# LuChengTHU/dpm-solver

Measured on NVIDIA H100. Metric: solver-update GElem/s, higher is better.
Workload: dtype bf16

## Files before the change

### dpm_solver_b200/_lib.py

```python
from __future__ import annotations

import ctypes as C
import os
from pathlib import Path

_PKG = Path(__file__).resolve().parent
LIB_PATH = _PKG / "lib" / "libdpmsolver_b200.so"

DPM_F32, DPM_BF16, DPM_F16 = 0, 1, 2
FORM_NONE, FORM_LIN1, FORM_LIN2, FORM_LIN3, FORM_DIFF2, FORM_MS3, FORM_SS3T = range(7)
PARAM_NOISE, PARAM_X_START, PARAM_V, PARAM_SCORE = range(4)

PARAM_BY_NAME = {"noise": PARAM_NOISE, "x_start": PARAM_X_START, "v": PARAM_V, "score": PARAM_SCORE}


class StepDesc(C.Structure):
    _fields_ = [
        ("x", C.c_void_p), ("xe", C.c_void_p), ("m0", C.c_void_p), ("m1", C.c_void_p),
        ("m2", C.c_void_p), ("m_out", C.c_void_p), ("out", C.c_void_p), ("out2", C.c_void_p),
        ("e_cond", C.c_void_p), ("e_uncond", C.c_void_p), ("thr", C.c_void_p),
        ("n", C.c_uint64), ("per_sample", C.c_uint64),
        ("state_dtype", C.c_int32), ("model_dtype", C.c_int32), ("form", C.c_int32),
        ("n_model", C.c_int32), ("param", C.c_int32), ("predict_x0", C.c_int32),
        ("c0_on_old", C.c_int32), ("raw_round", C.c_int32),
        ("guidance", C.c_float), ("alpha_e", C.c_float), ("sigma_e", C.c_float),
        ("a", C.c_float), ("c0", C.c_float), ("c1", C.c_float), ("c2", C.c_float),
        ("w0", C.c_float), ("w1", C.c_float), ("w2", C.c_float), ("w3", C.c_float),
        ("w4", C.c_float),
        ("dev_coef", C.c_void_p),
    ]


class AdaptiveCtl(C.Structure):
    _fields_ = [
        ("schedule_kind", C.c_int32), ("table_len", C.c_int32),
        ("t_array", C.c_void_p), ("log_alpha_array", C.c_void_p), ("log_alpha_flipped", C.c_void_p), ("t_flipped", C.c_void_p),
        ("beta_0", C.c_float), ("beta_1_minus_beta_0", C.c_float), ("inv_total_N", C.c_float),
        ("discrete_time_input", C.c_int32), ("order", C.c_int32), ("predict_x0", C.c_int32), ("taylor", C.c_int32),
        ("t_0", C.c_float), ("theta", C.c_float), ("t_err", C.c_float),
        ("state", C.c_void_p), ("coef", C.c_void_p), ("times", C.c_void_p), ("error", C.c_void_p),
    ]


_vp, _f, _u64, _i = C.c_void_p, C.c_float, C.c_uint64, C.c_int

PROTOTYPES = {
    "dpm_version": (C.c_int, []),
    "dpm_last_error": (C.c_char_p, []),
    "dpm_set_tuning": (C.c_int, [_i, _i, _i]),
    "dpm_get_tuning": (C.c_int, [C.POINTER(C.c_int)] * 3),
    "dpm_launch_count": (C.c_uint64, []),
    "dpm_step": (C.c_int, [C.POINTER(StepDesc), _vp]),
    "dpm_lincomb": (C.c_int, [_vp, _vp, _vp, _vp, _vp, _i, _f, _f, _f, _f, _u64, _i, _vp]),
    "dpm_solver_first_update": (C.c_int, [_vp, _vp, _vp, _f, _f, _u64, _i, _vp]),
    "dpm_multistep_second_update": (C.c_int, [_vp, _vp, _vp, _vp, _f, _f, _f, _f, _u64, _i, _vp]),
    "dpm_multistep_third_update": (C.c_int, [_vp] * 5 + [_f] * 8 + [_u64, _i, _vp]),
    "dpm_singlestep_diff_update": (C.c_int, [_vp, _vp, _vp, _vp, _f, _f, _f, _u64, _i, _vp]),
    "dpm_singlestep_third_taylor_update": (C.c_int, [_vp] * 5 + [_f] * 9 + [_u64, _i, _vp]),
    "dpm_cfg_combine": (C.c_int, [_vp, _vp, _vp, _f, _u64, _i, _vp]),
    "dpm_duplicate": (C.c_int, [_vp, _vp, _u64, _i, _vp]),
    "dpm_philox_policy": (C.c_int, [_u64, C.POINTER(C.c_uint32), C.POINTER(C.c_uint64)]),
    "dpm_add_noise_philox": (C.c_int, [_vp, _vp, _u64, _i, C.POINTER(C.c_float), C.POINTER(C.c_float), _u64, _u64, _i, _i, _vp]),
    "dpm_diffedit_corrector": (C.c_int, [_vp, _vp, _vp, _vp, _u64, _u64, _f, _f, _u64, _u64, _i, _vp]),
    "dpm_data_prediction": (C.c_int, [_vp, _vp, _vp, _f, _f, _vp, _u64, _u64, _i, _vp]),
    "dpm_dynamic_threshold_workspace": (C.c_size_t, [_u64, _u64]),
    "dpm_dynamic_threshold": (C.c_int, [_vp, C.POINTER(StepDesc), _f, _f, _vp, C.c_size_t, _vp]),
    "dpm_adaptive_init": (C.c_int, [C.POINTER(AdaptiveCtl), _f, _f, _vp]),
    "dpm_adaptive_plan": (C.c_int, [C.POINTER(AdaptiveCtl), _vp]),
    "dpm_adaptive_decide": (C.c_int, [C.POINTER(AdaptiveCtl), _vp]),
    "dpm_select_copy": (C.c_int, [_vp, _vp, _vp, _u64, _vp]),
    "dpm_adaptive_error_workspace": (C.c_size_t, [_u64, _u64]),
    "dpm_adaptive_error": (C.c_int, [_vp, _vp, _vp, _vp, _f, _f, _u64, _u64, _i, _vp, C.c_size_t, _vp]),
    "dpm_cfg_rescale_workspace": (C.c_size_t, [_u64, _u64]),
    "dpm_cfg_rescale_ratio": (C.c_int, [_vp, _vp, _vp, _f, _u64, _u64, _i, _vp, C.c_size_t, _vp]),
    "dpm_step_rescaled": (C.c_int, [C.POINTER(StepDesc), _vp, _f, _f, _vp]),
}

_lib = None


class DpmLibraryError(RuntimeError):
    pass


def lib() -> C.CDLL:
    global _lib
    if _lib is not None:
        return _lib
    path = Path(os.environ.get("DPM_B200_LIB", LIB_PATH))
    if not path.exists():
        raise DpmLibraryError(
            f"{path} not found. Build it with `python -m dpm_solver_b200.build` "
            "(needs nvcc, sm_90a). dpm_solver_b200 has no CPU or PyTorch fallback.")
    handle = C.CDLL(str(path))
    for name, (res, args) in PROTOTYPES.items():
        try:
            fn = getattr(handle, name)
        except AttributeError as e:
            raise DpmLibraryError(f"{path} does not export {name}") from e
        fn.restype = res
        fn.argtypes = args
    _lib = handle
    return _lib


def check(rc: int) -> None:
    if rc != 0:
        msg = lib().dpm_last_error().decode("utf-8", "replace")
        raise DpmLibraryError(f"libdpmsolver_b200 error {rc}: {msg}")
```

### dpm_solver_b200/csrc/capi.cu

```cuda
#include <atomic>
#include <mutex>
#include <set>
#include <utility>
#include <cstdarg>
#include <cstdio>
#include <cstdlib>
#include <cstring>

#include "launch.cuh"

namespace dpm {

static thread_local char g_err[512] = "";
static std::atomic<uint64_t> g_launches{0};
static std::atomic<int> g_variant{2}, g_threads{0}, g_ctas{0};

void set_error(const char* fmt, ...) {
  va_list ap;
  va_start(ap, fmt);
  vsnprintf(g_err, sizeof(g_err), fmt, ap);
  va_end(ap);
}
void count_launch() { g_launches.fetch_add(1, std::memory_order_relaxed); }
bool pdl_enabled() {
  static const bool on = [] { const char* e = getenv("DPM_PDL"); return !(e && e[0] == '0'); }();
  return on;
}

int launch_error(const char* what, cudaError_t e) {
  set_error("%s: %s", what, cudaGetErrorString(e));
  cudaGetLastError();
  return (int)e;
}

template <cudaDeviceAttr A, int FALLBACK>
static int device_attr() {
  static int cache[64] = {0};
  int dev = 0;
  if (cudaGetDevice(&dev) != cudaSuccess || dev < 0 || dev >= 64) return FALLBACK;
  if (cache[dev] == 0) {
    int v = 0;
    if (cudaDeviceGetAttribute(&v, A, dev) != cudaSuccess || v <= 0) v = FALLBACK;
    cache[dev] = v;
  }
  return cache[dev];
}
int sm_count() { return device_attr<cudaDevAttrMultiProcessorCount, 132>(); }
int max_smem_optin() { return device_attr<cudaDevAttrMaxSharedMemoryPerBlockOptin, 227 * 1024>(); }

int ensure_max_smem(const void* kernel, bool nonportable_cluster) {
  static std::mutex mu;
  static std::set<std::pair<int, const void*>> done;
  int dev = 0;
  cudaGetDevice(&dev);
  std::lock_guard<std::mutex> lock(mu);
  if (done.count({dev, kernel})) return 0;
  cudaFuncAttributes fa;
  cudaError_t e = cudaFuncGetAttributes(&fa, kernel);
  const int room = max_smem_optin() - (e == cudaSuccess ? (int)fa.sharedSizeBytes : 0);
  if (e == cudaSuccess) e = cudaFuncSetAttribute(kernel, cudaFuncAttributeMaxDynamicSharedMemorySize, room);
  if (e == cudaSuccess && nonportable_cluster)
    e = cudaFuncSetAttribute(kernel, cudaFuncAttributeNonPortableClusterSizeAllowed, 1);
  if (e != cudaSuccess) return launch_error("shared-memory opt-in failed", e);
  done.insert({dev, kernel});
  return 0;
}

static inline int esize(int dt) { return dt == DPM_F32 ? 4 : 2; }
static inline bool valid_dtype(int dt) { return dt == DPM_F32 || dt == DPM_BF16 || dt == DPM_F16; }
static inline bool aligned(const void* p, int dt) {
  const uintptr_t a = dt == DPM_F32 ? 32 : 16;
  return (reinterpret_cast<uintptr_t>(p) & (a - 1)) == 0;
}
static inline const void* off(const void* p, int dt, uint64_t elems) {
  return p ? static_cast<const char*>(p) + elems * esize(dt) : nullptr;
}
static inline void* off(void* p, int dt, uint64_t elems) {
  return p ? static_cast<char*>(p) + elems * esize(dt) : nullptr;
}

struct Needs {
  bool x, m0, m1, m2, ec, eu, xe;
};

static int build_params(const dpm_step_desc* d, KParams* kp, Needs* nd, bool for_quantile) {
  if (d == nullptr) { set_error("desc is NULL"); return DPM_ERR_ARG; }
  if (!valid_dtype(d->state_dtype) || !valid_dtype(d->model_dtype)) {
    set_error("bad dtype (state %d, model %d)", d->state_dtype, d->model_dtype);
    return DPM_ERR_ARG;
  }
  const int form = for_quantile ? DPM_FORM_NONE : d->form;
  if (form < DPM_FORM_NONE || form > DPM_FORM_SS3T) { set_error("bad form %d", form); return DPM_ERR_ARG; }
  if (d->n_model < 0 || d->n_model > 2) { set_error("n_model must be 0, 1 or 2"); return DPM_ERR_ARG; }
  if (d->param < DPM_PARAM_NOISE || d->param > DPM_PARAM_SCORE) { set_error("bad param %d", d->param); return DPM_ERR_ARG; }
  if (d->raw_round != 0 && ((d->raw_round & ~7) != 0 || ((d->raw_round & 3) != DPM_BF16 && (d->raw_round & 3) != DPM_F16))) {
    set_error("raw_round must be 0 or (DPM_BF16 | DPM_F16) [+ 4]");
    return DPM_ERR_ARG;
  }
  if (d->raw_round != 0 && (d->state_dtype != DPM_F32 || for_quantile)) {
    set_error("raw_round needs an fp32 state and is not available in dpm_dynamic_threshold");
    return DPM_ERR_ARG;
  }
  if ((d->n >> 3) > 0xffffffffull) { set_error("n too large (max 2^35-1 elements per call)"); return DPM_ERR_ARG; }

  const FormReads reads = form_reads(form);
  nd->x = reads.x;
  nd->m0 = d->n_model == 0;
  nd->m1 = reads.m1;
  nd->m2 = reads.m2;
// ... 57 lines not shown
static bool all_aligned(const KParams& p, const Needs& nd) {
  const int sd = p.state_dtype, md = p.model_dtype;
  bool ok = true;
  if (nd.x) ok &= aligned(p.x, sd);
  if (nd.xe) ok &= aligned(p.xe, sd);
  if (nd.m0) ok &= aligned(p.m0, sd);
  if (nd.m1) ok &= aligned(p.m1, sd);
  if (nd.m2) ok &= aligned(p.m2, sd);
  if (nd.ec) ok &= aligned(p.ec, md);
  if (nd.eu) ok &= aligned(p.eu, md);
  if (p.m_out) ok &= aligned(p.m_out, sd);
  if (p.out) ok &= aligned(p.out, sd);
  if (p.out2) ok &= aligned(p.out2, sd);
  return ok;
}

static KParams shifted(const KParams& p, uint64_t elems) {
  KParams t = p;
  const int sd = p.state_dtype, md = p.model_dtype;
  t.x = off(p.x, sd, elems); t.xe = off(p.xe, sd, elems); t.m0 = off(p.m0, sd, elems);
  t.m1 = off(p.m1, sd, elems); t.m2 = off(p.m2, sd, elems);
  t.ec = off(p.ec, md, elems); t.eu = off(p.eu, md, elems);
  t.m_out = off(p.m_out, sd, elems); t.out = off(p.out, sd, elems); t.out2 = off(p.out2, sd, elems);
  t.n = p.n - elems;
  t.elem_offset = elems;
  return t;
}

static int finish(int rc) {
  if (rc != DPM_OK) return rc;
  cudaError_t e = cudaPeekAtLastError();
  return e != cudaSuccess ? launch_error("CUDA launch failed", e) : DPM_OK;
}

struct Rescale {
  const float* ratio;
  float phi, psi;
};

static int step_impl(const dpm_step_desc* d, cudaStream_t stream, const Rescale* rs = nullptr) {
  KParams p;
  Needs nd;
  if (d != nullptr && d->n == 0) return DPM_OK;
  int rc = build_params(d, &p, &nd, false);
  if (rc != DPM_OK) return rc;
  if (p.n == 0) return DPM_OK;
  if (rs != nullptr) {
    if (rs->ratio == nullptr || d->n_model != 2 || d->raw_round != 0 || d->per_sample == 0 || d->n % d->per_sample) {
      set_error("rescaled step: needs ratio, n_model == 2, raw_round == 0 and per_sample dividing n");
      return DPM_ERR_ARG;
    }
    p.ratio = rs->ratio; p.phi = rs->phi; p.psi = rs->psi;
  }
  Tuning t{g_variant.load(), g_threads.load(), g_ctas.load()};

  bool body_done = false;
  if (p.npk > 0 && all_aligned(p, nd) && p.dev_coef == nullptr) {
    int r = 1;
    const bool tma = p.raw_round == 0 &&
                     p.ratio == nullptr &&
                     t.variant == 1;
    if (tma) r = launch_step_tma(p, t, stream);
    if (r == 1) r = launch_step_direct(p, t, stream);
    if (r < 0 || r > 1) return r;
    body_done = (r == 0);
  }
  if (!body_done) {
    rc = launch_step_scalar(p, stream);
  } else if (p.n % kPacket) {
    rc = launch_step_scalar(shifted(p, (uint64_t)p.npk * kPacket), stream);
  }
  return finish(rc);
}

}

using namespace dpm;

extern "C" {

int dpm_version(void) { return DPM_B200_VERSION; }
const char* dpm_last_error(void) { return g_err; }
uint64_t dpm_launch_count(void) { return g_launches.load(); }

int dpm_set_tuning(int variant, int threads, int ctas_per_sm) {
  if (variant < 0 || variant > 2) { set_error("variant must be 0 (direct), 1 (TMA ring) or 2 (auto)"); return DPM_ERR_ARG; }
  if (threads != 0 && (threads < 32 || threads > 512 || threads % 32)) { set_error("threads must be a multiple of 32 in [32,512]"); return DPM_ERR_ARG; }
  if (ctas_per_sm < 0 || ctas_per_sm > 32) { set_error("ctas_per_sm must be in [0,32]"); return DPM_ERR_ARG; }
  g_variant = variant; g_threads = threads; g_ctas = ctas_per_sm;
  return DPM_OK;
}
int dpm_get_tuning(int* variant, int* threads, int* ctas_per_sm) {
  if (variant) *variant = g_variant.load();
  if (threads) *threads = g_threads.load();
  if (ctas_per_sm) *ctas_per_sm = g_ctas.load();
  return DPM_OK;
}

int dpm_step(const dpm_step_desc* desc, dpm_stream_t stream) {
  return step_impl(desc, static_cast<cudaStream_t>(stream));
}

int dpm_step_rescaled(const dpm_step_desc* desc, const float* ratio, float phi, float one_minus_phi,
                      dpm_stream_t stream) {
  const Rescale rs{ratio, phi, one_minus_phi};
  return step_impl(desc, static_cast<cudaStream_t>(stream), &rs);
}

size_t dpm_cfg_rescale_workspace(uint64_t n_samples, uint64_t per_sample) {
  return cfg_rescale_workspace_bytes(n_samples, per_sample);
}

int dpm_cfg_rescale_ratio(float* ratio_out, const void* e_cond, const void* e_uncond, float guidance,
                          uint64_t per_sample, uint64_t n, int model_dtype, void* workspace, size_t workspace_bytes,
                          dpm_stream_t stream) {
  if (n == 0) return DPM_OK;
  if (!ratio_out || !e_cond || !e_uncond) { set_error("cfg rescale: NULL tensor"); return DPM_ERR_ARG; }
  if (!valid_dtype(model_dtype) || per_sample == 0 || n % per_sample) { set_error("cfg rescale: bad dtype or sizes"); return DPM_ERR_ARG; }
  return finish(launch_cfg_rescale_ratio(ratio_out, e_cond, e_uncond, guidance, per_sample, n, model_dtype, workspace,
                                         workspace_bytes, static_cast<cudaStream_t>(stream)));
}

static dpm_step_desc base_desc(void* out, const void* x, uint64_t n, int dtype, int form) {
  dpm_step_desc d;
  memset(&d, 0, sizeof(d));
  d.out = out; d.x = x; d.n = n; d.state_dtype = dtype; d.model_dtype = dtype; d.form = form;
  return d;
}

int dpm_lincomb(void* out, const void* x, const void* m0, const void* m1, const void* m2, int k,
                float a, float c0, float c1, float c2, uint64_t n, int dtype, dpm_stream_t stream) {
  if (k < 1 || k > 3) { set_error("k must be 1, 2 or 3"); return DPM_ERR_ARG; }
  dpm_step_desc d = base_desc(out, x, n, dtype, k == 1 ? DPM_FORM_LIN1 : k == 2 ? DPM_FORM_LIN2 : DPM_FORM_LIN3);
  d.m0 = m0; d.m1 = m1; d.m2 = m2; d.a = a; d.c0 = c0; d.c1 = c1; d.c2 = c2;
  return dpm_step(&d, stream);
}

int dpm_solver_first_update(void* x_t, const void* x, const void* model_s, float a, float c0,
                            uint64_t n, int dtype, dpm_stream_t stream) {
  dpm_step_desc d = base_desc(x_t, x, n, dtype, DPM_FORM_LIN1);
  d.m0 = model_s; d.a = a; d.c0 = c0;
  return dpm_step(&d, stream);
}

int dpm_multistep_second_update(void* x_t, const void* x, const void* model_prev_0,
                                const void* model_prev_1, float a, float c0, float c1,
                                float inv_r0, uint64_t n, int dtype, dpm_stream_t stream) {
  dpm_step_desc d = base_desc(x_t, x, n, dtype, DPM_FORM_DIFF2);
  d.m0 = model_prev_0; d.m1 = model_prev_1; d.a = a; d.c0 = c0; d.c1 = c1; d.w0 = inv_r0;
  return dpm_step(&d, stream);
}

int dpm_multistep_third_update(void* x_t, const void* x, const void* model_prev_0,
                               const void* model_prev_1, const void* model_prev_2, float a,
                               float c0, float c1, float c2, float inv_r0, float inv_r1, float w,
                               float q, uint64_t n, int dtype, dpm_stream_t stream) {
  dpm_step_desc d = base_desc(x_t, x, n, dtype, DPM_FORM_MS3);
  d.m0 = model_prev_0; d.m1 = model_prev_1; d.m2 = model_prev_2;
  d.a = a; d.c0 = c0; d.c1 = c1; d.c2 = c2; d.w0 = inv_r0; d.w1 = inv_r1; d.w2 = w; d.w3 = q;
  return dpm_step(&d, stream);
}

int dpm_singlestep_diff_update(void* x_t, const void* x, const void* model_s,
                               const void* model_new, float a, float c0, float c1, uint64_t n,
                               int dtype, dpm_stream_t stream) {
  dpm_step_desc d = base_desc(x_t, x, n, dtype, DPM_FORM_DIFF2);
// ... 117 lines not shown
```

### dpm_solver_b200/csrc/common.cuh

```cuda
#pragma once
#include <cuda_bf16.h>
#include <cuda_fp16.h>
#include <cuda_runtime.h>
#include <stdint.h>
#include <string.h>

#include "dpm_solver_b200.h"

namespace dpm {

constexpr int kPacket = 8;

struct KParams {
  const void* x;
  const void* xe;
  const void* m0;
  const void* m1;
  const void* m2;
  const void* ec;
  const void* eu;
  void* m_out;
  void* out;
  void* out2;
  const float* thr;
  uint64_t n;
  uint32_t npk;
  uint32_t pk_per_sample;
  uint64_t per_sample;
  uint64_t elem_offset;
  int32_t param;
  int32_t predict_x0;
  int32_t c0_on_old;
  int32_t use_xe;
  int32_t xe_is_x;
  int32_t form;
  int32_t n_model;
  int32_t state_dtype;
  int32_t model_dtype;
  float guidance, alpha_e, sigma_e;
  float a, c0, c1, c2;
  float w0, w1, w2, w3, w4;
  float r_alpha;
  int32_t raw_round;
  float r_w4;
  int32_t fast_div;
  const float* dev_coef;
  const float* ratio;
  float phi, psi;
};

template <typename T> struct Raw;
template <> struct Raw<float> { uint32_t r[8]; };
template <> struct Raw<__nv_bfloat16> { uint32_t r[4]; };
template <> struct Raw<__half> { uint32_t r[4]; };

template <typename T> struct Traits;
template <> struct Traits<float> { static constexpr int kBytes = 4; static constexpr int kCode = DPM_F32; };
template <> struct Traits<__nv_bfloat16> { static constexpr int kBytes = 2; static constexpr int kCode = DPM_BF16; };
template <> struct Traits<__half> { static constexpr int kBytes = 2; static constexpr int kCode = DPM_F16; };

__device__ __forceinline__ void ldg_pk(Raw<float>& v, const float* p) {
  asm volatile("ld.global.L1::no_allocate.v4.b32 {%0,%1,%2,%3}, [%8];\n\t"
               "ld.global.L1::no_allocate.v4.b32 {%4,%5,%6,%7}, [%8+16];"
               : "=r"(v.r[0]), "=r"(v.r[1]), "=r"(v.r[2]), "=r"(v.r[3]), "=r"(v.r[4]),
                 "=r"(v.r[5]), "=r"(v.r[6]), "=r"(v.r[7])
               : "l"(p));
}
template <typename T16>
__device__ __forceinline__ void ldg_pk(Raw<T16>& v, const T16* p) {
  asm volatile("ld.global.L1::no_allocate.v4.b32 {%0,%1,%2,%3}, [%4];"
               : "=r"(v.r[0]), "=r"(v.r[1]), "=r"(v.r[2]), "=r"(v.r[3])
               : "l"(p));
}
__device__ __forceinline__ void stg_pk(float* p, const Raw<float>& v) {
  asm volatile("st.global.L1::no_allocate.v4.b32 [%0], {%1,%2,%3,%4};\n\t"
               "st.global.L1::no_allocate.v4.b32 [%0+16], {%5,%6,%7,%8};" ::"l"(p),
               "r"(v.r[0]), "r"(v.r[1]), "r"(v.r[2]), "r"(v.r[3]), "r"(v.r[4]), "r"(v.r[5]),
               "r"(v.r[6]), "r"(v.r[7])
               : "memory");
}
template <typename T16>
__device__ __forceinline__ void stg_pk(T16* p, const Raw<T16>& v) {
  asm volatile("st.global.L1::no_allocate.v4.b32 [%0], {%1,%2,%3,%4};" ::"l"(p), "r"(v.r[0]),
               "r"(v.r[1]), "r"(v.r[2]), "r"(v.r[3])
               : "memory");
}

__device__ __forceinline__ void unpack(const Raw<float>& v, float (&f)[8]) {
#pragma unroll
  for (int i = 0; i < 8; ++i) f[i] = __uint_as_float(v.r[i]);
}
__device__ __forceinline__ void unpack(const Raw<__nv_bfloat16>& v, float (&f)[8]) {
#pragma unroll
  for (int i = 0; i < 4; ++i) {
    f[2 * i] = __uint_as_float(v.r[i] << 16);
    f[2 * i + 1] = __uint_as_float(v.r[i] & 0xffff0000u);
  }
}
__device__ __forceinline__ void unpack(const Raw<__half>& v, float (&f)[8]) {
#pragma unroll
  for (int i = 0; i < 4; ++i) {
    __half2 h = *reinterpret_cast<const __half2*>(&v.r[i]);
    float2 t = __half22float2(h);
    f[2 * i] = t.x;
    f[2 * i + 1] = t.y;
  }
}
__device__ __forceinline__ void pack(Raw<float>& v, const float (&f)[8]) {
#pragma unroll
  for (int i = 0; i < 8; ++i) v.r[i] = __float_as_uint(f[i]);
}
__device__ __forceinline__ void pack(Raw<__nv_bfloat16>& v, const float (&f)[8]) {
#pragma unroll
  for (int i = 0; i < 4; ++i) {
    __nv_bfloat162 h = __floats2bfloat162_rn(f[2 * i], f[2 * i + 1]);
    v.r[i] = *reinterpret_cast<uint32_t*>(&h);
  }
}
__device__ __forceinline__ void pack(Raw<__half>& v, const float (&f)[8]) {
#pragma unroll
  for (int i = 0; i < 4; ++i) {
    __half2 h = __floats2half2_rn(f[2 * i], f[2 * i + 1]);
    v.r[i] = *reinterpret_cast<uint32_t*>(&h);
  }
}

template <typename T> __device__ __forceinline__ float round_storage(float v);
template <> __device__ __forceinline__ float round_storage<float>(float v) { return v; }
template <> __device__ __forceinline__ float round_storage<__nv_bfloat16>(float v) {
  return __bfloat162float(__float2bfloat16_rn(v));
}
// ... 250 lines not shown
```

### dpm_solver_b200/csrc/launch.cuh

```cuda
#pragma once
#include <cuda_runtime.h>
#include <stdint.h>

#include <type_traits>

#include "common.cuh"

namespace dpm {

struct Tuning {
  int variant;
  int threads;
  int ctas_per_sm;
};

int sm_count();
int max_smem_optin();
void count_launch();
int ensure_max_smem(const void* kernel, bool nonportable_cluster = false);
void set_error(const char* fmt, ...);
int launch_error(const char* what, cudaError_t e);

template <typename TE_, typename TS_> struct PacketPair {
  using TE = TE_;
  using TS = TS_;
};
template <typename F>
static inline auto with_packet_pair(int md, int sd, F&& f) -> decltype(f(PacketPair<float, float>{})) {
  if (md == DPM_F32 && sd == DPM_F32) return f(PacketPair<float, float>{});
  if (md == DPM_BF16 && sd == DPM_BF16) return f(PacketPair<__nv_bfloat16, __nv_bfloat16>{});
  if (md == DPM_F16 && sd == DPM_F16) return f(PacketPair<__half, __half>{});
  if (md == DPM_BF16 && sd == DPM_F32) return f(PacketPair<__nv_bfloat16, float>{});
  if (md == DPM_F16 && sd == DPM_F32) return f(PacketPair<__half, float>{});
  return {};
}
template <typename F>
static inline auto with_form(int form, F&& f) -> decltype(f(std::integral_constant<int, DPM_FORM_NONE>{})) {
  switch (form) {
    case DPM_FORM_NONE: return f(std::integral_constant<int, DPM_FORM_NONE>{});
    case DPM_FORM_LIN1: return f(std::integral_constant<int, DPM_FORM_LIN1>{});
    case DPM_FORM_LIN2: return f(std::integral_constant<int, DPM_FORM_LIN2>{});
    case DPM_FORM_LIN3: return f(std::integral_constant<int, DPM_FORM_LIN3>{});
    case DPM_FORM_DIFF2: return f(std::integral_constant<int, DPM_FORM_DIFF2>{});
    case DPM_FORM_MS3: return f(std::integral_constant<int, DPM_FORM_MS3>{});
    case DPM_FORM_SS3T: return f(std::integral_constant<int, DPM_FORM_SS3T>{});
  }
  return {};
}
template <typename R, typename Pick>
static inline R pick_step(const KParams& p, Pick&& pick) {
  const int md = p.n_model == 0 ? p.state_dtype : p.model_dtype;
  return with_packet_pair(md, p.state_dtype, [&](auto pair) -> R {
    return with_form(p.form, [&](auto form) -> R {
      using Pair = decltype(pair);
      switch (p.n_model) {
        case 0:
          if constexpr (decltype(form)::value != DPM_FORM_NONE && std::is_same_v<typename Pair::TE, typename Pair::TS>)
            return pick(pair, std::integral_constant<int, 0>{}, form);
          return R{};
        case 1: return pick(pair, std::integral_constant<int, 1>{}, form);
        case 2: return pick(pair, std::integral_constant<int, 2>{}, form);
      }
      return R{};
    });
  });
}

__device__ __forceinline__ void pdl_trigger() { asm volatile("griddepcontrol.launch_dependents;" ::: "memory"); }
__device__ __forceinline__ void pdl_wait() { asm volatile("griddepcontrol.wait;" ::: "memory"); }
bool pdl_enabled();

template <typename... KArgs, typename... Args>
static inline cudaError_t launch_pdl(void (*kernel)(KArgs...), unsigned grid, unsigned block, size_t smem, cudaStream_t stream,
                                     Args&&... args) {
  cudaLaunchConfig_t cfg;
  memset(&cfg, 0, sizeof(cfg));
  cfg.gridDim = dim3(grid, 1, 1);
  cfg.blockDim = dim3(block, 1, 1);
  cfg.dynamicSmemBytes = smem;
  cfg.stream = stream;
  cudaLaunchAttribute attr[1];
  attr[0].id = cudaLaunchAttributeProgrammaticStreamSerialization;
  attr[0].val.programmaticStreamSerializationAllowed = 1;
  cfg.attrs = attr;
  cfg.numAttrs = pdl_enabled() ? 1 : 0;
  return cudaLaunchKernelEx(&cfg, kernel, static_cast<KArgs>(args)...);
}

int launch_step_direct(const KParams& p, const Tuning& t, cudaStream_t stream);
int launch_step_scalar(const KParams& p, cudaStream_t stream);
int launch_step_tma(const KParams& p, const Tuning& t, cudaStream_t stream);
void philox_policy(uint64_t numel, uint32_t* grid, uint64_t* counter_offset);
int launch_noise_philox(void* out, const void* x, const void* xt, const float* mask, uint64_t mask_n, uint64_t n,
                        int t_count, const float* alpha, const float* sigma, uint64_t seed, uint64_t offset,
                        int x_dtype, int out_dtype, cudaStream_t stream);
int launch_adaptive_init(const dpm_adaptive_ctl* a, float t_T, float h_init, cudaStream_t stream);
int launch_adaptive_plan(const dpm_adaptive_ctl* a, cudaStream_t stream);
int launch_adaptive_decide(const dpm_adaptive_ctl* a, cudaStream_t stream);
int launch_select_copy(void* dst, const void* src, const float* state, uint64_t bytes, cudaStream_t stream);
int launch_duplicate(void* dst, const void* src, uint64_t bytes, cudaStream_t stream);
int launch_quantile(float* s_out, const KParams& p, uint64_t n_samples, float q, float max_val,
                    void* workspace, size_t workspace_bytes, cudaStream_t stream);
size_t quantile_workspace_bytes(uint64_t n_samples, uint64_t per_sample);
size_t adaptive_workspace_bytes(uint64_t n, uint64_t per_sample);
int launch_adaptive_error(float* out, const void* xh, const void* xl, const void* xp, float atol, float rtol,
                          uint64_t per_sample, uint64_t n, int dtype, void* ws, size_t ws_bytes, cudaStream_t stream);
size_t cfg_rescale_workspace_bytes(uint64_t n_samples, uint64_t per_sample);
int launch_cfg_rescale_ratio(float* ratio, const void* ec, const void* eu, float guidance, uint64_t per_sample,
                             uint64_t n, int dtype, void* ws, size_t ws_bytes, cudaStream_t stream);

}
```

### dpm_solver_b200/csrc/step_direct.cu

```cuda
#include "common.cuh"
#include "launch.cuh"

namespace dpm {

constexpr int kUnroll = 2;
constexpr int kMaxThreads = 512;

template <typename TE, typename TS, int NE, int FORM, bool FAST, bool RND = false, bool RS = false>
__global__ void __launch_bounds__(kMaxThreads)
    k_step_direct(const __grid_constant__ KParams p) {
  constexpr bool kX = form_reads(FORM).x, kM1 = form_reads(FORM).m1, kM2 = form_reads(FORM).m2;
  const TS* __restrict__ gx = static_cast<const TS*>(p.x);
  const TS* __restrict__ gxe = static_cast<const TS*>(p.xe);
  const TS* __restrict__ gm0 = static_cast<const TS*>(p.m0);
  const TS* __restrict__ gm1 = static_cast<const TS*>(p.m1);
  const TS* __restrict__ gm2 = static_cast<const TS*>(p.m2);
  const TE* __restrict__ gec = static_cast<const TE*>(p.ec);
  const TE* __restrict__ geu = static_cast<const TE*>(p.eu);
  TS* __restrict__ gmo = static_cast<TS*>(p.m_out);
  TS* __restrict__ go = static_cast<TS*>(p.out);
  TS* __restrict__ go2 = static_cast<TS*>(p.out2);

  const uint32_t npk = p.npk;
  const uint32_t tile_pk = blockDim.x * kUnroll;
  const bool sep_xe = (NE > 0) && p.use_xe && !(kX && p.xe_is_x);
  const bool clamp = (NE > 0) && (p.thr != nullptr);
  pdl_trigger();
  pdl_wait();

  for (uint64_t tile0 = (uint64_t)blockIdx.x * tile_pk; tile0 < npk;
       tile0 += (uint64_t)gridDim.x * tile_pk) {
    Raw<TS> rx[kUnroll], rxe[kUnroll], rm0[kUnroll], rm1[kUnroll], rm2[kUnroll];
    Raw<TE> rec[kUnroll], reu[kUnroll];
#pragma unroll
    for (int u = 0; u < kUnroll; ++u) {
      const uint64_t pk = tile0 + (uint64_t)u * blockDim.x + threadIdx.x;
      if (pk < npk) {
        const size_t e = (size_t)pk * kPacket;
        if (kX) ldg_pk(rx[u], gx + e);
        if (NE > 0) {
          ldg_pk(rec[u], gec + e);
          if (NE == 2) ldg_pk(reu[u], geu + e);
          if (sep_xe) ldg_pk(rxe[u], gxe + e);
        } else {
          ldg_pk(rm0[u], gm0 + e);
        }
        if (kM1) ldg_pk(rm1[u], gm1 + e);
        if (kM2) ldg_pk(rm2[u], gm2 + e);
      }
    }
#pragma unroll
    for (int u = 0; u < kUnroll; ++u) {
      const uint64_t pk = tile0 + (uint64_t)u * blockDim.x + threadIdx.x;
      if (pk < npk) {
        const size_t e = (size_t)pk * kPacket;
        float fx[8], fxe[8], fT[8], fm1[8], fm2[8], fo[8];
        if (kX) unpack(rx[u], fx);
        if (kM1) unpack(rm1[u], fm1);
        if (kM2) unpack(rm2[u], fm2);
        if (NE > 0 && FAST) {
          float fec[8], feu[8];
          unpack(rec[u], fec);
          if (NE == 2) unpack(reu[u], feu);
          const float s_thr = clamp ? __ldg(p.thr + (uint32_t)pk / p.pk_per_sample) : 1.f;
          const float r = RS ? __ldg(p.ratio + (uint32_t)pk / p.pk_per_sample) : 1.f;
          if (sep_xe) {
            unpack(rxe[u], fxe);
            fast_model8<NE, RS>(p, fxe, fec, feu, clamp, s_thr, fT, r);
          } else {
            fast_model8<NE, RS>(p, fx, fec, feu, clamp, s_thr, fT, r);
          }
          Raw<TS> rmo;
          round_pack(rmo, fT);
          if (gmo != nullptr) stg_pk(gmo + e, rmo);
        } else if (NE > 0) {
          float fec[8], feu[8];
          unpack(rec[u], fec);
          if (NE == 2) unpack(reu[u], feu);
          if (sep_xe) {
            unpack(rxe[u], fxe);
          } else if (kX) {
#pragma unroll
            for (int i = 0; i < 8; ++i) fxe[i] = fx[i];
          } else {
#pragma unroll
            for (int i = 0; i < 8; ++i) fxe[i] = 0.f;
          }
          float thr8[8];
          const bool thr_uniform = p.pk_per_sample != 0;
          if (clamp) {
            if (thr_uniform) {
              const float tpk = __ldg(p.thr + (uint32_t)(pk / p.pk_per_sample));
#pragma unroll
              for (int i = 0; i < 8; ++i) thr8[i] = tpk;
            } else {
#pragma unroll
              for (int i = 0; i < 8; ++i) thr8[i] = __ldg(p.thr + (e + i) / p.per_sample);
            }
          } else {
#pragma unroll
            for (int i = 0; i < 8; ++i) thr8[i] = 1.f;
          }
          float r8[8];
#pragma unroll
          for (int i = 0; i < 8; ++i) r8[i] = 1.f;
          if (RS) {
            if (thr_uniform) {
              const float rpk = __ldg(p.ratio + (uint32_t)(pk / p.pk_per_sample));
#pragma unroll
              for (int i = 0; i < 8; ++i) r8[i] = rpk;
            } else {
#pragma unroll
              for (int i = 0; i < 8; ++i) r8[i] = __ldg(p.ratio + (e + i) / p.per_sample);
            }
// ... 34 lines not shown
    p.a = c[0]; p.c0 = c[1]; p.c1 = c[2]; p.c2 = c[3];
    p.w0 = c[4]; p.w1 = c[5]; p.w2 = c[6]; p.w3 = c[7]; p.w4 = c[8];
    p.alpha_e = c[9]; p.sigma_e = c[10];
    p.fast_div = 0;
  }
  const int sd = p.state_dtype, md = p.model_dtype;
  const FormReads reads = form_reads(p.form);
  const bool need_x = reads.x, need_m1 = reads.m1, need_m2 = reads.m2;
  const bool clamp = p.n_model > 0 && p.thr != nullptr;
  for (size_t i = (size_t)blockIdx.x * blockDim.x + threadIdx.x; i < p.n;
       i += (size_t)gridDim.x * blockDim.x) {
    float x = need_x ? load_any(p.x, sd, i) : 0.f;
    float m1 = need_m1 ? load_any(p.m1, sd, i) : 0.f;
    float m2 = need_m2 ? load_any(p.m2, sd, i) : 0.f;
    float T0;
    if (p.n_model > 0) {
      float xe = p.use_xe ? ((need_x && p.xe_is_x) ? x : load_any(p.xe, sd, i)) : 0.f;
      float ec = load_any(p.ec, md, i);
      float eu = p.n_model == 2 ? load_any(p.eu, md, i) : 0.f;
      float thr = clamp ? p.thr[(i + p.elem_offset) / p.per_sample] : 1.f;
      float mv;
      if (RS) {
        mv = model_value<2, false, true>(p, xe, ec, eu, thr, clamp, p.ratio[(i + p.elem_offset) / p.per_sample]);
      } else {
        mv = p.n_model == 2 ? model_value<2, RND>(p, xe, ec, eu, thr, clamp)
                            : model_value<1, RND>(p, xe, ec, eu, thr, clamp);
      }
      T0 = round_any(sd, mv);
      if (p.m_out) store_any(p.m_out, sd, i, mv);
    } else {
      T0 = load_any(p.m0, sd, i);
    }
    float o;
    switch (p.form) {
      case DPM_FORM_LIN1: o = update_value<DPM_FORM_LIN1, RND>(p, x, T0, m1, m2); break;
      case DPM_FORM_LIN2: o = update_value<DPM_FORM_LIN2, RND>(p, x, T0, m1, m2); break;
      case DPM_FORM_LIN3: o = update_value<DPM_FORM_LIN3, RND>(p, x, T0, m1, m2); break;
      case DPM_FORM_DIFF2: o = update_value<DPM_FORM_DIFF2, RND>(p, x, T0, m1, m2); break;
      case DPM_FORM_MS3: o = update_value<DPM_FORM_MS3, RND>(p, x, T0, m1, m2); break;
      case DPM_FORM_SS3T: o = update_value<DPM_FORM_SS3T, RND>(p, x, T0, m1, m2); break;
      default: continue;
    }
    store_any(p.out, sd, i, o);
    if (p.out2) store_any(p.out2, sd, i, o);
  }
}

typedef void (*StepKernel)(const KParams);

static StepKernel pick_direct(const KParams& p) {
  const bool fast = fast_path_ok(p), rnd = p.raw_round != 0, rs = p.ratio != nullptr;
  return pick_step<StepKernel>(p, [&](auto pair, auto ne, auto form) -> StepKernel {
    using TE = typename decltype(pair)::TE;
    using TS = typename decltype(pair)::TS;
    constexpr int NE = decltype(ne)::value, FORM = decltype(form)::value;
    if (rs) {
      if constexpr (NE == 2)
        return fast ? k_step_direct<TE, TS, 2, FORM, true, false, true> : k_step_direct<TE, TS, 2, FORM, false, false, true>;
      else
        return nullptr;
    }
    if (rnd) {
      if constexpr (std::is_same_v<TS, float> && (NE == 0) == std::is_same_v<TE, float>)
        return k_step_direct<TE, TS, NE, FORM, false, true>;
      else
        return nullptr;
    }
    if constexpr (NE == 0 && FORM != DPM_FORM_SS3T)
      return k_step_direct<TE, TS, NE, FORM, true>;
    else
      return fast ? k_step_direct<TE, TS, NE, FORM, true> : k_step_direct<TE, TS, NE, FORM, false>;
  });
}

int launch_step_direct(const KParams& p, const Tuning& t, cudaStream_t stream) {
  StepKernel k = pick_direct(p);
  if (k == nullptr) return 1;
  const int threads = t.threads > 0 ? t.threads : 256;
  const uint32_t tile_pk = (uint32_t)threads * kUnroll;
  uint64_t tiles = ((uint64_t)p.npk + tile_pk - 1) / tile_pk;
  uint64_t cap = t.ctas_per_sm > 0 ? (uint64_t)sm_count() * t.ctas_per_sm : tiles;
  uint32_t grid = (uint32_t)(tiles < cap ? tiles : cap);
  if (grid == 0) return 0;
  cudaError_t le = launch_pdl(k, grid, (unsigned)threads, 0, stream, p);
  if (le != cudaSuccess) return launch_error("step launch failed", le);
  count_launch();
  return 0;
}

int launch_step_scalar(const KParams& p, cudaStream_t stream) {
  if (p.n == 0) return 0;
  const int threads = 256;
  uint64_t blocks = (p.n + threads - 1) / threads;
  uint64_t cap = (uint64_t)sm_count() * 8;
  uint32_t grid = (uint32_t)(blocks < cap ? blocks : cap);
  if (p.raw_round) k_step_scalar<true><<<grid, threads, 0, stream>>>(p);
  else if (p.ratio) k_step_scalar<false, true><<<grid, threads, 0, stream>>>(p);
  else k_step_scalar<false><<<grid, threads, 0, stream>>>(p);
  count_launch();
  return 0;
}

}
```

### dpm_solver_b200/ops.py

```python
from __future__ import annotations

import ctypes as C
from dataclasses import dataclass
from typing import Optional, Tuple

import torch

from . import _lib
from ._lib import (DPM_BF16, DPM_F16, DPM_F32, FORM_DIFF2, FORM_LIN1, FORM_LIN2, FORM_LIN3,
                   FORM_MS3, FORM_NONE, FORM_SS3T, PARAM_NOISE, StepDesc)

_DTYPE_CODE = {torch.float32: DPM_F32, torch.bfloat16: DPM_BF16, torch.float16: DPM_F16}
SUPPORTED_DTYPES = tuple(_DTYPE_CODE)


@dataclass
class StepArgs:
    form: int = FORM_NONE
    n_model: int = 0
    x: Optional[torch.Tensor] = None
    xe: Optional[torch.Tensor] = None
    m0: Optional[torch.Tensor] = None
    m1: Optional[torch.Tensor] = None
    m2: Optional[torch.Tensor] = None
# ... 220 lines not shown
    def error_norm(self, x_higher, x_lower, x_prev, atol: float, rtol: float, out=None) -> torch.Tensor:
        n, dev = x_higher.numel(), x_higher.device
        ts = [self._check(t, w, dev, n, x_higher.dtype) for t, w in ((x_higher, "x_higher"), (x_lower, "x_lower"), (x_prev, "x_prev"))]
        per_sample = n // x_higher.shape[0]
        if out is None:
            out = torch.empty(1, dtype=torch.float32, device=dev)
        ws_bytes = int(self._lib.dpm_adaptive_error_workspace(n, per_sample))
        ws = torch.empty(max(ws_bytes, 4), dtype=torch.uint8, device=dev)
        self._launch(dev, self._lib.dpm_adaptive_error, C.c_void_p(out.data_ptr()), C.c_void_p(ts[0].data_ptr()),
                     C.c_void_p(ts[1].data_ptr()), C.c_void_p(ts[2].data_ptr()), C.c_float(atol), C.c_float(rtol),
                     C.c_uint64(per_sample), C.c_uint64(n), C.c_int(_DTYPE_CODE[x_higher.dtype]),
                     C.c_void_p(ws.data_ptr()), C.c_size_t(ws_bytes))
        return out

    def duplicate(self, x: torch.Tensor) -> torch.Tensor:
        if x.dtype not in _DTYPE_CODE:
            return torch.cat([x] * 2)
        layout = self._layout(x)
        if layout is None:
            x, layout = x.contiguous(), "c"
        shape = (2 * x.shape[0],) + tuple(x.shape[1:])
        if layout == "cl":
            out = torch.empty(shape, dtype=x.dtype, device=x.device,
                              memory_format=torch.channels_last if x.dim() == 4 else torch.channels_last_3d)
        else:
            out = torch.empty(shape, dtype=x.dtype, device=x.device)
        self._check(x, "x", x.device, x.numel(), layout=layout)
        self._launch(x.device, self._lib.dpm_duplicate, C.c_void_p(out.data_ptr()), C.c_void_p(x.data_ptr()),
                     C.c_uint64(x.numel()), C.c_int(_DTYPE_CODE[x.dtype]))
        return out

    def adaptive_controller(self, ns, device, **kw) -> "AdaptiveController":
        return AdaptiveController(self, ns, device, **kw)

    @staticmethod
    def _philox_state(device, numel: int, lib, generator=None):
        gen = generator if generator is not None else torch.cuda.default_generators[device.index]
        grid, inc = C.c_uint32(0), C.c_uint64(0)
        _lib.check(lib.dpm_philox_policy(C.c_uint64(numel), C.byref(grid), C.byref(inc)))
        seed, offset = gen.initial_seed(), gen.get_offset()
        gen.set_offset(offset + inc.value)
        return seed, offset

    def add_noise_philox(self, x: torch.Tensor, alphas, sigmas, out_dtype, generator=None) -> torch.Tensor:
        if torch.cuda.is_current_stream_capturing():
            raise RuntimeError("dpm_solver_b200: in-kernel noise reads the generator state on the host; pass `noise=` under CUDA-graph capture")
        x = self._check(x, "x", x.device, x.numel())
        T = len(alphas)
        out = torch.empty((T,) + tuple(x.shape), dtype=out_dtype, device=x.device)
        with torch.cuda.device(x.device):
            seed, offset = self._philox_state(x.device, T * x.numel(), self._lib, generator)
        fa = (C.c_float * T)(*alphas)
        fs = (C.c_float * T)(*sigmas)
        self._launch(x.device, self._lib.dpm_add_noise_philox, C.c_void_p(out.data_ptr()), C.c_void_p(x.data_ptr()),
                     C.c_uint64(x.numel()), C.c_int(T), fa, fs, C.c_uint64(seed), C.c_uint64(offset),
                     C.c_int(_DTYPE_CODE[x.dtype]), C.c_int(_DTYPE_CODE[out_dtype]))
        return out

    def diffedit_corrector(self, x, x0, mask, alpha: float, sigma: float, generator=None) -> torch.Tensor:
        if torch.cuda.is_current_stream_capturing():
            raise RuntimeError("dpm_solver_b200: in-kernel noise reads the generator state on the host; not capturable")
        n = x.numel()
        x = self._check(x, "x", x.device, n)
        x0 = self._check(x0, "x0", x.device, n, x.dtype)
        if mask.dtype != torch.float32 or not mask.is_contiguous() or n % max(mask.numel(), 1) \
                or tuple(mask.shape) != tuple(x.shape[x.dim() - mask.dim():]):
            mask = mask.to(torch.float32).expand(x.shape).contiguous()
        if mask.device != x.device:
            raise RuntimeError("dpm_solver_b200: `mask` must live on the device of x")
        out = torch.empty_like(x)
        with torch.cuda.device(x.device):
            seed, offset = self._philox_state(x.device, n, self._lib, generator)
        self._launch(x.device, self._lib.dpm_diffedit_corrector, C.c_void_p(out.data_ptr()), C.c_void_p(x.data_ptr()),
                     C.c_void_p(x0.data_ptr()), C.c_void_p(mask.data_ptr()), C.c_uint64(mask.numel()), C.c_uint64(n),
                     C.c_float(alpha), C.c_float(sigma), C.c_uint64(seed), C.c_uint64(offset), C.c_int(_DTYPE_CODE[x.dtype]))
        return out

    def prepare(self, a: StepArgs) -> Optional["PreparedStep"]:
        return PreparedStep.build(self, a)

    def launch_count(self) -> int:
        return int(self._lib.dpm_launch_count())

    def set_tuning(self, variant: int = 2, threads: int = 0, ctas_per_sm: int = 0) -> None:
        _lib.check(self._lib.dpm_set_tuning(variant, threads, ctas_per_sm))


class AdaptiveController:

    SUPPORTED = ("discrete", "linear")

    def __init__(self, be: "CudaBackend", ns, device, order: int, predict_x0: bool, taylor: bool, t_0: float,
                 theta: float, t_err: float, discrete_input: bool):
        if ns.schedule not in self.SUPPORTED:
            raise ValueError("the device controller supports the 'discrete' and 'linear' schedules")
        self.be, self.dev = be, torch.device(device)
        f32 = dict(dtype=torch.float32, device=self.dev)
        self.state = torch.zeros(16, **f32)
        self.coef = torch.zeros(4, 16, **f32)
        self.times = torch.zeros(6, **f32)
        self.E = torch.zeros(1, **f32)
        c = self.ctl = _lib.AdaptiveCtl()
        self._keep = []
        if ns.schedule == "discrete":
            tabs = ns._table(self.dev)[:4]
            self._keep = [t.to(torch.float32).contiguous() for t in tabs]
            c.schedule_kind, c.table_len = 0, self._keep[0].numel()
            c.t_array, c.log_alpha_array, c.log_alpha_flipped, c.t_flipped = (t.data_ptr() for t in self._keep)
            c.inv_total_N = 1. / ns.total_N
        else:
            c.schedule_kind, c.table_len = 1, 0
            c.beta_0, c.beta_1_minus_beta_0 = ns.beta_0, ns.beta_1 - ns.beta_0
            c.inv_total_N = 1. / ns.total_N
        c.discrete_time_input = int(bool(discrete_input))
        c.order, c.predict_x0, c.taylor = order, int(bool(predict_x0)), int(bool(taylor))
        c.t_0, c.theta, c.t_err = t_0, theta, t_err
        c.state, c.coef, c.times, c.error = (t.data_ptr() for t in (self.state, self.coef, self.times, self.E))
        self._ref = C.byref(c)

    def init(self, t_T: float, h_init: float) -> None:
        self.be._launch(self.dev, self.be._lib.dpm_adaptive_init, self._ref, C.c_float(t_T), C.c_float(h_init))

    def plan(self) -> None:
        self.be._launch(self.dev, self.be._lib.dpm_adaptive_plan, self._ref)

    def decide(self) -> None:
        self.be._launch(self.dev, self.be._lib.dpm_adaptive_decide, self._ref)

    def select_copy(self, dst: torch.Tensor, src: torch.Tensor) -> None:
        if dst.shape != src.shape or dst.dtype != src.dtype or not dst.is_contiguous() or not src.is_contiguous():
            raise ValueError("select_copy: dense tensors of one shape and dtype")
        self.be._launch(self.dev, self.be._lib.dpm_select_copy, C.c_void_p(dst.data_ptr()), C.c_void_p(src.data_ptr()),
                        C.c_void_p(self.state.data_ptr()), C.c_uint64(dst.numel() * dst.element_size()))

    def block(self, i: int) -> torch.Tensor:
        return self.coef[i]

    def time(self, j: int) -> torch.Tensor:
        return self.times[j:j + 1]

    def input_time(self, j: int) -> torch.Tensor:
        return self.times[3 + j:4 + j]

    def read(self):
        st = self.state.cpu().view(torch.int32)
        return int(st[6]), int(st[5]), int(st[8])


class PreparedStep:

    __slots__ = ("be", "d", "ref_d", "fn", "n", "dev", "dev_index", "sdt", "mdt", "shape", "shape2", "need_out",
                 "need_m", "fields", "dup", "ptrs", "esize")

    ORDER = ("x", "xe", "m0", "m1", "m2", "e_cond", "e_uncond")
    _PTR = {"x": 0, "xe": 1, "m0": 2, "m1": 3, "m2": 4, "m_out": 5, "out": 6, "out2": 7, "e_cond": 8, "e_uncond": 9}

    @staticmethod
    def build(be: "CudaBackend", a: StepArgs) -> Optional["PreparedStep"]:
        if a.thr is not None or a.raw_round or a.ratio is not None or a.out is not None and a.out2 is None:
            return None
        ref = a.reference_tensor()
        if not ref.is_contiguous():
            return None
        for t in a.state_tensors() + a.model_tensors():
            if not t.is_contiguous() or t.device != ref.device:
                return None
# ... 87 lines not shown
```

### include/dpm_solver_b200.h

```cpp
#ifndef DPM_SOLVER_B200_H
#define DPM_SOLVER_B200_H

#include <stddef.h>
#include <stdint.h>

#ifdef __cplusplus
extern "C" {
#endif

#define DPM_B200_VERSION 100

#if defined(__GNUC__)
#define DPM_API __attribute__((visibility("default")))
#else
#define DPM_API
#endif

typedef void* dpm_stream_t;

typedef enum dpm_status {
  DPM_OK = 0,
  DPM_ERR_ARG = -1,
  DPM_ERR_UNSUPPORTED = -2,
  DPM_ERR_ALIGN = -3
} dpm_status;

typedef enum dpm_dtype { DPM_F32 = 0, DPM_BF16 = 1, DPM_F16 = 2 } dpm_dtype;

typedef enum dpm_form {
  DPM_FORM_NONE = 0,
  DPM_FORM_LIN1 = 1,
  DPM_FORM_LIN2 = 2,
  DPM_FORM_LIN3 = 3,
  DPM_FORM_DIFF2 = 4,
  DPM_FORM_MS3 = 5,
  DPM_FORM_SS3T = 6
} dpm_form;

typedef enum dpm_param {
  DPM_PARAM_NOISE = 0,
  DPM_PARAM_X_START = 1,
  DPM_PARAM_V = 2,
  DPM_PARAM_SCORE = 3
} dpm_param;

typedef struct dpm_step_desc {
  const void* x;
  const void* xe;
  const void* m0;
  const void* m1;
  const void* m2;
  void* m_out;
  void* out;
  void* out2;
  const void* e_cond;
  const void* e_uncond;
  const float* thr;
  uint64_t n;
  uint64_t per_sample;
  int32_t state_dtype;
  int32_t model_dtype;
  int32_t form;
  int32_t n_model;
  int32_t param;
  int32_t predict_x0;
  int32_t c0_on_old;
  int32_t raw_round;
  float guidance;
  float alpha_e;
  float sigma_e;
  float a, c0, c1, c2;
  float w0, w1, w2, w3, w4;
  const float* dev_coef;
} dpm_step_desc;

DPM_API int dpm_version(void);
DPM_API const char* dpm_last_error(void);

DPM_API int dpm_set_tuning(int variant, int threads, int ctas_per_sm);
DPM_API int dpm_get_tuning(int* variant, int* threads, int* ctas_per_sm);
DPM_API uint64_t dpm_launch_count(void);

DPM_API int dpm_step(const dpm_step_desc* desc, dpm_stream_t stream);


DPM_API int dpm_lincomb(void* out, const void* x, const void* m0, const void* m1, const void* m2,
                int k, float a, float c0, float c1, float c2, uint64_t n, int dtype,
                dpm_stream_t stream);

DPM_API int dpm_solver_first_update(void* x_t, const void* x, const void* model_s, float a, float c0,
                            uint64_t n, int dtype, dpm_stream_t stream);

DPM_API int dpm_multistep_second_update(void* x_t, const void* x, const void* model_prev_0,
                                const void* model_prev_1, float a, float c0, float c1,
                                float inv_r0, uint64_t n, int dtype, dpm_stream_t stream);

DPM_API int dpm_multistep_third_update(void* x_t, const void* x, const void* model_prev_0,
                               const void* model_prev_1, const void* model_prev_2, float a,
                               float c0, float c1, float c2, float inv_r0, float inv_r1,
                               float w, float q, uint64_t n, int dtype, dpm_stream_t stream);

DPM_API int dpm_singlestep_diff_update(void* x_t, const void* x, const void* model_s,
                               const void* model_new, float a, float c0, float c1, uint64_t n,
                               int dtype, dpm_stream_t stream);

DPM_API int dpm_singlestep_third_taylor_update(void* x_t, const void* x, const void* model_s,
                                       const void* model_s1, const void* model_s2, float a,
                                       float c0, float c1, float c2, float inv_r1, float inv_r2,
                                       float r2, float r1, float r2_minus_r1, uint64_t n,
                                       int dtype, dpm_stream_t stream);

DPM_API int dpm_cfg_combine(void* eps, const void* eps_uncond, const void* eps_cond, float scale,
                    uint64_t n, int dtype, dpm_stream_t stream);

DPM_API int dpm_duplicate(void* out, const void* x, uint64_t n, int dtype, dpm_stream_t stream);

DPM_API int dpm_data_prediction(void* x0, const void* x, const void* eps, float alpha_t, float sigma_t,
                        const float* thr, uint64_t per_sample, uint64_t n, int dtype,
                        dpm_stream_t stream);

DPM_API int dpm_philox_policy(uint64_t numel, uint32_t* grid, uint64_t* counter_offset);

DPM_API int dpm_add_noise_philox(void* xt, const void* x, uint64_t n, int t_count, const float* alpha_t,
                                 const float* sigma_t, uint64_t seed, uint64_t offset, int x_dtype, int out_dtype,
                                 dpm_stream_t stream);

DPM_API int dpm_diffedit_corrector(void* out, const void* x, const void* x0, const float* mask, uint64_t mask_n,
                                   uint64_t n, float alpha_t, float sigma_t, uint64_t seed, uint64_t offset,
                                   int dtype, dpm_stream_t stream);

DPM_API size_t dpm_dynamic_threshold_workspace(uint64_t n_samples, uint64_t per_sample);
DPM_API int dpm_dynamic_threshold(float* s_out, const dpm_step_desc* desc, float q, float max_val,
                                  void* workspace, size_t workspace_bytes, dpm_stream_t stream);

DPM_API size_t dpm_adaptive_error_workspace(uint64_t n, uint64_t per_sample);
DPM_API int dpm_adaptive_error(float* e_out, const void* x_higher, const void* x_lower,
                               const void* x_prev, float atol, float rtol, uint64_t per_sample,
                               uint64_t n, int dtype, void* workspace, size_t workspace_bytes,
                               dpm_stream_t stream);

DPM_API size_t dpm_cfg_rescale_workspace(uint64_t n_samples, uint64_t per_sample);
DPM_API int dpm_cfg_rescale_ratio(float* ratio_out, const void* e_cond, const void* e_uncond, float guidance,
                                  uint64_t per_sample, uint64_t n, int model_dtype,
                                  void* workspace, size_t workspace_bytes, dpm_stream_t stream);
DPM_API int dpm_step_rescaled(const dpm_step_desc* desc, const float* ratio, float phi, float one_minus_phi,
                              dpm_stream_t stream);

typedef struct dpm_adaptive_ctl {
  int32_t schedule_kind;
  int32_t table_len;
  const float* t_array;
  const float* log_alpha_array;
  const float* log_alpha_flipped;
  const float* t_flipped;
  float beta_0, beta_1_minus_beta_0, inv_total_N;
  int32_t discrete_time_input;
  int32_t order;
  int32_t predict_x0;
  int32_t taylor;
  float t_0, theta, t_err;
  float* state;
  float* coef;
  float* times;
  const float* error;
// ... 12 lines not shown
```

Baseline: 305.6.

## Reverse tile traversal when a step consumes the previous step's output for L2 reuse

Keeps a per-device/stream record of each step launch's output pointers. When the next launch reads one of them, the direct kernel walks its tiles in reverse order, so the tail written last, still likely resident in L2, is read first. Consecutive dependent launches alternate direction. This adds host-side mutex and map bookkeeping per launch, plus a subtraction in the tile loop, and it only affects the direct kernel variant.

```diff
diff --git a/dpm_solver_b200/_lib.py b/dpm_solver_b200/_lib.py
--- a/dpm_solver_b200/_lib.py
+++ b/dpm_solver_b200/_lib.py
@@ -50,6 +50,7 @@
     "dpm_set_tuning": (C.c_int, [_i, _i, _i]),
     "dpm_get_tuning": (C.c_int, [C.POINTER(C.c_int)] * 3),
     "dpm_launch_count": (C.c_uint64, []),
+    "dpm_reversed_launch_count": (C.c_uint64, []),
     "dpm_step": (C.c_int, [C.POINTER(StepDesc), _vp]),
     "dpm_lincomb": (C.c_int, [_vp, _vp, _vp, _vp, _vp, _i, _f, _f, _f, _f, _u64, _i, _vp]),
     "dpm_solver_first_update": (C.c_int, [_vp, _vp, _vp, _f, _f, _u64, _i, _vp]),
diff --git a/dpm_solver_b200/csrc/capi.cu b/dpm_solver_b200/csrc/capi.cu
--- a/dpm_solver_b200/csrc/capi.cu
+++ b/dpm_solver_b200/csrc/capi.cu
@@ -1,6 +1,9 @@
 #include <atomic>
+#include <map>
 #include <mutex>
 #include <set>
+#include <thread>
+#include <tuple>
 #include <utility>
 #include <cstdarg>
 #include <cstdio>
@@ -25,6 +28,34 @@
 bool pdl_enabled() {
   static const bool on = [] { const char* e = getenv("DPM_PDL"); return !(e && e[0] == '0'); }();
   return on;
+}
+
+static std::atomic<uint64_t> g_reversed{0};
+
+bool l2_carry(const KParams& p, cudaStream_t stream) {
+  static const bool on = [] { const char* e = getenv("DPM_L2_CARRY"); return !(e && e[0] == '0'); }();
+  if (!on) return false;
+  struct Last {
+    const void *out, *m_out, *out2;
+    bool reverse;
+  };
+  static std::mutex mu;
+  static std::map<std::tuple<int, cudaStream_t, std::thread::id>, Last> last;
+  int dev = 0;
+  cudaGetDevice(&dev);
+  const std::thread::id tid = stream == cudaStreamPerThread ? std::this_thread::get_id() : std::thread::id();
+  const FormReads r = form_reads(p.form);
+  const void* in[5] = {r.x ? p.x : nullptr, p.use_xe ? p.xe : nullptr, p.n_model == 0 ? p.m0 : nullptr,
+                       r.m1 ? p.m1 : nullptr, r.m2 ? p.m2 : nullptr};
+  std::lock_guard<std::mutex> lock(mu);
+  if (last.size() >= 4096) last.clear();
+  Last& l = last[{dev, stream, tid}];
+  bool follows = false;
+  for (const void* q : in) follows |= q != nullptr && (q == l.out || q == l.m_out || q == l.out2);
+  const bool reverse = follows && !l.reverse;
+  l = {p.form != DPM_FORM_NONE ? p.out : nullptr, p.m_out, p.out2, reverse};
+  if (reverse) g_reversed.fetch_add(1, std::memory_order_relaxed);
+  return reverse;
 }
 
 int launch_error(const char* what, cudaError_t e) {
@@ -248,6 +279,7 @@
 int dpm_version(void) { return DPM_B200_VERSION; }
 const char* dpm_last_error(void) { return g_err; }
 uint64_t dpm_launch_count(void) { return g_launches.load(); }
+uint64_t dpm_reversed_launch_count(void) { return g_reversed.load(); }
 
 int dpm_set_tuning(int variant, int threads, int ctas_per_sm) {
   if (variant < 0 || variant > 2) { set_error("variant must be 0 (direct), 1 (TMA ring) or 2 (auto)"); return DPM_ERR_ARG; }
diff --git a/dpm_solver_b200/csrc/common.cuh b/dpm_solver_b200/csrc/common.cuh
--- a/dpm_solver_b200/csrc/common.cuh
+++ b/dpm_solver_b200/csrc/common.cuh
@@ -47,6 +47,7 @@
   const float* dev_coef;
   const float* ratio;
   float phi, psi;
+  uint64_t rev_pk0;
 };
 
 template <typename T> struct Raw;
diff --git a/dpm_solver_b200/csrc/launch.cuh b/dpm_solver_b200/csrc/launch.cuh
--- a/dpm_solver_b200/csrc/launch.cuh
+++ b/dpm_solver_b200/csrc/launch.cuh
@@ -69,6 +69,7 @@
 __device__ __forceinline__ void pdl_trigger() { asm volatile("griddepcontrol.launch_dependents;" ::: "memory"); }
 __device__ __forceinline__ void pdl_wait() { asm volatile("griddepcontrol.wait;" ::: "memory"); }
 bool pdl_enabled();
+bool l2_carry(const KParams& p, cudaStream_t stream);
 
 template <typename... KArgs, typename... Args>
 static inline cudaError_t launch_pdl(void (*kernel)(KArgs...), unsigned grid, unsigned block, size_t smem, cudaStream_t stream,
diff --git a/dpm_solver_b200/csrc/step_direct.cu b/dpm_solver_b200/csrc/step_direct.cu
--- a/dpm_solver_b200/csrc/step_direct.cu
+++ b/dpm_solver_b200/csrc/step_direct.cu
@@ -28,8 +28,8 @@
   pdl_trigger();
   pdl_wait();
 
-  for (uint64_t tile0 = (uint64_t)blockIdx.x * tile_pk; tile0 < npk;
-       tile0 += (uint64_t)gridDim.x * tile_pk) {
+  for (uint64_t t0 = (uint64_t)blockIdx.x * tile_pk; t0 < npk; t0 += (uint64_t)gridDim.x * tile_pk) {
+    const uint64_t tile0 = p.rev_pk0 ? p.rev_pk0 - t0 : t0;
     Raw<TS> rx[kUnroll], rxe[kUnroll], rm0[kUnroll], rm1[kUnroll], rm2[kUnroll];
     Raw<TE> rec[kUnroll], reu[kUnroll];
 #pragma unroll
@@ -230,7 +230,9 @@
   uint64_t cap = t.ctas_per_sm > 0 ? (uint64_t)sm_count() * t.ctas_per_sm : tiles;
   uint32_t grid = (uint32_t)(tiles < cap ? tiles : cap);
   if (grid == 0) return 0;
-  cudaError_t le = launch_pdl(k, grid, (unsigned)threads, 0, stream, p);
+  KParams q = p;
+  q.rev_pk0 = l2_carry(p, stream) ? (tiles - 1) * tile_pk : 0;
+  cudaError_t le = launch_pdl(k, grid, (unsigned)threads, 0, stream, q);
   if (le != cudaSuccess) return launch_error("step launch failed", le);
   count_launch();
   return 0;
diff --git a/dpm_solver_b200/ops.py b/dpm_solver_b200/ops.py
--- a/dpm_solver_b200/ops.py
+++ b/dpm_solver_b200/ops.py
@@ -326,6 +326,9 @@
     def launch_count(self) -> int:
         return int(self._lib.dpm_launch_count())
 
+    def reversed_launch_count(self) -> int:
+        return int(self._lib.dpm_reversed_launch_count())
+
     def set_tuning(self, variant: int = 2, threads: int = 0, ctas_per_sm: int = 0) -> None:
         _lib.check(self._lib.dpm_set_tuning(variant, threads, ctas_per_sm))
 
diff --git a/include/dpm_solver_b200.h b/include/dpm_solver_b200.h
--- a/include/dpm_solver_b200.h
+++ b/include/dpm_solver_b200.h
@@ -80,6 +80,7 @@
 DPM_API int dpm_set_tuning(int variant, int threads, int ctas_per_sm);
 DPM_API int dpm_get_tuning(int* variant, int* threads, int* ctas_per_sm);
 DPM_API uint64_t dpm_launch_count(void);
+DPM_API uint64_t dpm_reversed_launch_count(void);
 
 DPM_API int dpm_step(const dpm_step_desc* desc, dpm_stream_t stream);
 
```

Result: faster. 310.6 (median of 6 runs) (+1.6%).
